# pengpeng-yu/FastPCC

Hardware: NVIDIA B200
Metric: encode+decode Mpts/s (higher is better)
Workload: dtype int8

## Files before the change

### fastpcc_b200/_lib.py

```python
import ctypes as C
import os.path as osp

from . import build as _build

_vp, _i, _i64, _sz = C.c_void_p, C.c_int, C.c_int64, C.c_size_t


class Epilogue(C.Structure):
    _fields_ = [('bias', _vp), ('slope', _vp), ('requant_mul', _vp), ('zero_point', _vp),
                ('shift', C.c_int32), ('out_type', C.c_int32), ('mul_is_scalar', C.c_int32),
                ('residual', _vp), ('post_slope', _vp), ('row_bias', _vp), ('row_idx', _vp), ('row_bias_bound', C.c_int32),
                ('post_requant_mul', _vp), ('post_zero_point', _vp), ('post_shift', C.c_int32), ('post_requant_slope', _vp), ('aux_out', _vp), ('out_ld', C.c_int64)]


_EP = C.POINTER(Epilogue)

SIGNATURES = {
    'fpcc_last_error': (C.c_char_p, []),
    'fpcc_version': (_i, []),
    'fpcc_device_check': (_i, [_vp, _vp, _vp]),
    'fpcc_hash_insert_coords': (_i, [_vp, _vp, _i, _vp, _i, _i, _vp]),
    'fpcc_kmap_lookup': (_i, [_vp, _vp, _i, _vp, _i, _i, _i, _i, _i, _i, _i, _i, _i, _vp, _i, _i64, _vp]),
    'fpcc_kmap_compact_workspace': (_sz, [_i, _i]),
    'fpcc_kmap_compact': (_i, [_vp, _i, _i, _i64, _i, _vp, _vp, _vp, _vp, _sz, _vp]),
    'fpcc_kmap_from_parent': (_i, [_vp, _i64, _i, _vp, _vp, _vp, _vp, _i, _vp, _i64, _vp]),
    'fpcc_kmap_row_masks': (_i, [_vp, _i, _i, _i64, _vp, _vp]),
    'fpcc_kmap_permute': (_i, [_vp, _i, _i, _i64, _vp, _vp, _i64, _vp]),
    'fpcc_scan_workspace': (_sz, [_i]),
    'fpcc_downsample': (_i, [_vp, _i, _vp, _vp, _vp, _vp, _vp, _vp, _sz, _vp]),
    'fpcc_upsample': (_i, [_vp, _vp, _i, _vp, _vp, _vp, _vp, _vp, _vp, _sz, _vp]),
    'fpcc_occ_to_bits': (_i, [_vp, _i, _vp, _vp]),
    'fpcc_gather_patches': (_i, [_vp, _i, _vp, _i64, _i, _i, _vp, _i, _vp]),
    'fpcc_occ_bits_q8': (_i, [_vp, _i64, _i, _i, _vp, _i64, _vp]),
    'fpcc_slot_table': (_i, [_vp, _vp, _i, _vp, _i64, _vp]),
    'fpcc_morton_encode': (_i, [_vp, _i64, _i, _i, _vp, _vp]),
    'fpcc_gather_rows16': (_i, [_vp, _vp, _i64, _vp, _vp]),
    'fpcc_voxelize_workspace': (_sz, [_i64]),
    'fpcc_voxelize_f32': (_i, [_vp, _i64, _i, C.c_float, _i, _i, _i, _vp, _vp, _vp, _vp, _sz, _vp]),
    'fpcc_kd_split_workspace': (_sz, [_i64, _i]),
    'fpcc_kd_split': (_i, [_vp, _i64, _i, _vp, _vp, _vp, _sz, _vp]),
    'fpcc_frame_header_write': (_i, [_vp, _i, _vp]),
    'fpcc_frame_header_read': (_i, [_vp, _i64, _vp, _vp]),
    'fpcc_partitions_pack': (_i64, [_vp, _vp, _i, _vp, _i64]),
    'fpcc_partitions_index': (_i, [_vp, _i64, _i, _vp, _vp]),
    'fpcc_bytes_list_concat': (_i64, [_vp, _vp, _i, _vp, _i64]),
    'fpcc_bytes_list_split': (_i64, [_vp, _i64, _i, _vp, _vp]),
    'fpcc_nn_search': (_i, [_vp, _i, _i, _i, _vp, _i, _i, _i, _i, _vp, _vp, _vp]),
    'fpcc_knn_workspace': (_sz, [_i64, _i]),
    'fpcc_knn_search': (_i, [_i, _i, _i, _vp, _i64, _i, _i, _i, _vp, _i64, _i, _i, _i, _vp, _vp, _vp, _sz, _vp]),
    'fpcc_gemm_i8': (_i, [_vp, _vp, _vp, _i, _vp, _i, _i, _i, _vp]),
# ... 64 lines not shown
```

### fastpcc_b200/csrc/coords.cu

```cuda
#include <cub/cub.cuh>

#include "common.cuh"

namespace fpcc {


__device__ __forceinline__ int4 load_bxyz(const int32_t *coords, int64_t i, int layout) {
    int4 c = reinterpret_cast<const int4 *>(coords)[i];
    return layout == 0 ? c : make_int4(c.w, c.x, c.y, c.z);
}

__global__ void __launch_bounds__(256) hash_insert_kernel(unsigned long long *keys, int32_t *vals, uint32_t capacity,
                                                          const int32_t *coords, int n, int layout) {
    int i = blockIdx.x * blockDim.x + threadIdx.x;
    if (i >= n) return;
    int4 c = load_bxyz(coords, i, layout);
    if (!coord_in_range(c.x, c.y, c.z, c.w)) return;
    unsigned long long key = pack_key(c.x, c.y, c.z, c.w);
    uint32_t slot = hash_slot(key, capacity);
    while (true) {
        unsigned long long prev = atomicCAS(&keys[slot], 0ull, key);
        if (prev == 0ull || prev == key) {
            vals[slot] = i + 1;
            return;
// ... 43 lines not shown
    }
    dx = d[0]; dy = d[1]; dz = d[2];
}

__global__ void __launch_bounds__(256) kmap_lookup_kernel(const unsigned long long *__restrict__ keys,
                                                          const int32_t *__restrict__ vals, uint32_t capacity,
                                                          const int32_t *__restrict__ out_coords, int n_out, int layout,
                                                          KernelGeom g, int32_t *__restrict__ table, int k_major, int64_t ld) {
    int o = blockIdx.x * blockDim.x + threadIdx.x;
    int k = blockIdx.y;
    if (o >= n_out) return;
    int dx, dy, dz;
    kernel_offset(g, k, dx, dy, dz);
    int4 c = load_bxyz(out_coords, o, layout);
    int x, y, z;
    if (g.me) { x = c.y + dx; y = c.z + dy; z = c.w + dz; }
    else { x = c.y * g.st[0] + dx; y = c.z * g.st[1] + dy; z = c.w * g.st[2] + dz; }
    int32_t v = 0;
    if (coord_in_range(c.x, x, y, z)) v = hash_find(keys, vals, capacity, pack_key(c.x, x, y, z));
    if (k_major) table[(int64_t)k * ld + o] = v;
    else table[(int64_t)o * g.kvol + k] = v;
}

__global__ void __launch_bounds__(256) kmap_from_parent_kernel(const int32_t *__restrict__ ctable, int64_t ldc,
                                                               const uint8_t *__restrict__ cocc, const int32_t *__restrict__ cbase,
                                                               const int32_t *__restrict__ parent, const uint8_t *__restrict__ slot,
                                                               int n_fine, int32_t *__restrict__ table, int64_t ld) {
    const int i = blockIdx.x * blockDim.x + threadIdx.x;
    if (i >= n_fine) return;
    const int j = parent[i];
    const int s = slot[i];
    const int sx = (s >> 2) & 1, sy = (s >> 1) & 1, sz = s & 1;
    uint32_t pocc[8];
    int32_t pbase[8];
#pragma unroll
    for (int q = 0; q < 8; ++q) {
        const int K = (sx + (q & 1)) + 3 * (sy + ((q >> 1) & 1)) + 9 * (sz + (q >> 2));
        const int32_t jn = __ldg(&ctable[(int64_t)K * ldc + j]);
        pocc[q] = jn ? (uint32_t)__ldg(&cocc[jn - 1]) : 0u;
        pbase[q] = jn ? __ldg(&cbase[jn - 1]) : 0;
    }
#pragma unroll
    for (int dz = -1; dz <= 1; ++dz) {
        const int tz = sz + dz;
        const bool cz = ((tz >> 1) - (sz - 1)) != 0;
        uint32_t o4[4];
        int32_t b4[4];
#pragma unroll
        for (int q = 0; q < 4; ++q) { o4[q] = cz ? pocc[4 + q] : pocc[q]; b4[q] = cz ? pbase[4 + q] : pbase[q]; }
#pragma unroll
        for (int dy = -1; dy <= 1; ++dy) {
            const int ty = sy + dy;
            const bool cy = ((ty >> 1) - (sy - 1)) != 0;
            const uint32_t o2a = cy ? o4[2] : o4[0], o2b = cy ? o4[3] : o4[1];
            const int32_t b2a = cy ? b4[2] : b4[0], b2b = cy ? b4[3] : b4[1];
#pragma unroll
            for (int dx = -1; dx <= 1; ++dx) {
                const int tx = sx + dx;
                const bool cx = ((tx >> 1) - (sx - 1)) != 0;
                const uint32_t o = cx ? o2b : o2a;
                const int32_t b = cx ? b2b : b2a;
                const int sn = ((tx & 1) << 2) | ((ty & 1) << 1) | (tz & 1);
                const int32_t v = ((o >> (7 - sn)) & 1u) ? b + __popc(o >> (8 - sn)) + 1 : 0;
                const int k = (dx + 1) + 3 * (dy + 1) + 9 * (dz + 1);
                table[(int64_t)k * ld + i] = v;
            }
        }
    }
}

__global__ void __launch_bounds__(256) kmap_row_masks_kernel(const int32_t *__restrict__ table, int kvol, int n_out, int64_t ld,
                                                             int32_t *__restrict__ masks) {
    int o = blockIdx.x * blockDim.x + threadIdx.x;
    if (o >= n_out) return;
    uint32_t m = 0;
    for (int k = 0; k < kvol; ++k) m |= (uint32_t)(table[(int64_t)k * ld + o] != 0) << (k < 31 ? k : 31);
    masks[o] = (int32_t)(m & 0x7FFFFFFFu);
}
__global__ void __launch_bounds__(256) kmap_permute_kernel(const int32_t *__restrict__ table, int n_out, int64_t ld,
                                                           const int32_t *__restrict__ perm, int32_t *__restrict__ out, int64_t ld_out) {
    int j = blockIdx.x * blockDim.x + threadIdx.x;
    int k = blockIdx.y;
    if (j >= n_out) return;
    out[(int64_t)k * ld_out + j] = table[(int64_t)k * ld + perm[j]];
}

constexpr int CHUNK = 2048;

__global__ void __launch_bounds__(256) compact_count_kernel(const int32_t *__restrict__ table, int n_out, int64_t ld,
                                                            int omit_k, int nchunks, int32_t *__restrict__ counts) {
    int k = blockIdx.y, chunk = blockIdx.x;
    int base = chunk * CHUNK;
    int c = 0;
    if (k != omit_k) {
        for (int j = threadIdx.x; j < CHUNK; j += 256) {
            int o = base + j;
            if (o < n_out && table[(int64_t)k * ld + o] != 0) ++c;
        }
    }
    typedef cub::BlockReduce<int, 256> BR;
    __shared__ typename BR::TempStorage tmp;
    int tot = BR(tmp).Sum(c);
    if (threadIdx.x == 0) counts[k * nchunks + chunk] = tot;
}

__global__ void __launch_bounds__(256) compact_write_kernel(const int32_t *__restrict__ table, int n_out, int64_t ld,
                                                            int omit_k, int nchunks, const int32_t *__restrict__ starts,
// ... 145 lines not shown
                                int32_t *table, int k_major, int64_t ld, void *stream) {
    FPCC_REQUIRE(keys && vals && out_coords && table, "kmap_lookup: NULL pointer");
    FPCC_REQUIRE(ksx > 0 && ksy > 0 && ksz > 0 && sx > 0 && sy > 0 && sz > 0, "kmap_lookup: bad kernel geometry");
    FPCC_REQUIRE(capacity > 0 && n_out >= 0, "kmap_lookup: bad sizes");
    FPCC_REQUIRE(!k_major || ld >= n_out, "kmap_lookup: ld %lld < n_out %d", (long long)ld, n_out);
    FPCC_REQUIRE(((uintptr_t)out_coords & 15) == 0, "kmap_lookup: coords must be 16-byte aligned");
    if (n_out == 0) return FPCC_OK;
    KernelGeom g;
    g.ks[0] = ksx; g.ks[1] = ksy; g.ks[2] = ksz;
    g.st[0] = sx; g.st[1] = sy; g.st[2] = sz;
    g.kvol = ksx * ksy * ksz;
    g.me = convention == 1;
    FPCC_REQUIRE(convention == 0 || convention == 1, "kmap_lookup: unknown convention");
    FPCC_REQUIRE(g.kvol <= 65535, "kmap_lookup: kernel volume too large");
    dim3 grid(ceil_div(n_out, 256), g.kvol);
    kmap_lookup_kernel<<<grid, 256, 0, (cudaStream_t)stream>>>((const unsigned long long *)keys, vals, (uint32_t)capacity,
                                                               out_coords, n_out, layout, g, table, k_major, ld);
    FPCC_LAUNCH_CHECK();
    return FPCC_OK;
}

extern "C" int fpcc_kmap_from_parent(const int32_t *coarse_table, int64_t ld_coarse, int n_coarse, const uint8_t *coarse_occ,
                                     const int32_t *child_base, const int32_t *parent, const uint8_t *slot, int n_fine,
                                     int32_t *table, int64_t ld, void *stream) {
    FPCC_REQUIRE(coarse_table && coarse_occ && child_base && parent && slot && table, "kmap_from_parent: NULL pointer");
    FPCC_REQUIRE(n_coarse > 0 && ld_coarse >= n_coarse && n_fine >= 0 && ld >= n_fine, "kmap_from_parent: bad sizes");
    if (n_fine == 0) return FPCC_OK;
    kmap_from_parent_kernel<<<ceil_div(n_fine, 256), 256, 0, (cudaStream_t)stream>>>(coarse_table, ld_coarse, coarse_occ, child_base,
                                                                                                  parent, slot, n_fine, table, ld);
    FPCC_LAUNCH_CHECK();
    return FPCC_OK;
}

extern "C" int fpcc_kmap_row_masks(const int32_t *table, int kvol, int n_out, int64_t ld, int32_t *masks, void *stream) {
    FPCC_REQUIRE(table && masks, "kmap_row_masks: NULL pointer");
    FPCC_REQUIRE(kvol > 0 && n_out >= 0 && ld >= n_out, "kmap_row_masks: bad sizes");
    if (n_out == 0) return FPCC_OK;
    kmap_row_masks_kernel<<<ceil_div(n_out, 256), 256, 0, (cudaStream_t)stream>>>(table, kvol, n_out, ld, masks);
    FPCC_LAUNCH_CHECK();
    return FPCC_OK;
}

extern "C" int fpcc_kmap_permute(const int32_t *table, int kvol, int n_out, int64_t ld, const int32_t *perm, int32_t *out,
                                 int64_t ld_out, void *stream) {
    FPCC_REQUIRE(table && perm && out, "kmap_permute: NULL pointer");
    FPCC_REQUIRE(kvol > 0 && kvol <= 65535 && n_out >= 0 && ld >= n_out && ld_out >= n_out, "kmap_permute: bad sizes");
    if (n_out == 0) return FPCC_OK;
    kmap_permute_kernel<<<dim3(ceil_div(n_out, 256), kvol), 256, 0, (cudaStream_t)stream>>>(table, n_out, ld, perm, out, ld_out);
    FPCC_LAUNCH_CHECK();
    return FPCC_OK;
}

static size_t scan_temp_bytes(int n) {
    size_t t = 0;
    cub::DeviceScan::ExclusiveSum((void *)nullptr, t, (const int32_t *)nullptr, (int32_t *)nullptr, n);
    return (t + 255) & ~(size_t)255;
}

extern "C" size_t fpcc_kmap_compact_workspace(int kvol, int n_out) {
    int nchunks = ceil_div(n_out > 0 ? n_out : 1, CHUNK);
    size_t cnt = ((size_t)kvol * nchunks * sizeof(int32_t) + 255) & ~(size_t)255;
    return 2 * cnt + scan_temp_bytes(kvol * nchunks) + 256;
}

extern "C" int fpcc_kmap_compact(const int32_t *table, int kvol, int n_out, int64_t ld, int omit_k, int32_t *in_map,
                                 int32_t *out_map, int32_t *offsets, void *workspace, size_t workspace_bytes, void *stream) {
    FPCC_REQUIRE(table && in_map && out_map && offsets && workspace, "kmap_compact: NULL pointer");
    FPCC_REQUIRE(kvol > 0 && n_out > 0 && ld >= n_out, "kmap_compact: bad sizes");
    FPCC_REQUIRE(workspace_bytes >= fpcc_kmap_compact_workspace(kvol, n_out), "kmap_compact: workspace too small");
    cudaStream_t s = (cudaStream_t)stream;
    int nchunks = ceil_div(n_out, CHUNK);
// ... 203 lines not shown
```

### fastpcc_b200/csrc/entropy.cu

```cuda
#include "common.cuh"

namespace fpcc {

constexpr int EXP_LUT_SIZE = 12 * 512 + 1;
__device__ const int32_t g_exp_lut[EXP_LUT_SIZE] = {
#include "exp_lut.inc"
};

__device__ __forceinline__ int32_t warp_max(int32_t v) {
    return __reduce_max_sync(0xffffffffu, v);
}
__device__ __forceinline__ int32_t warp_sum(int32_t v) {
    return __reduce_add_sync(0xffffffffu, v);
}

struct RowStat {
    int32_t row_max;
    uint64_t inv;
};
__device__ __forceinline__ int32_t lut_of(int32_t row_max, int32_t x) {
    int32_t id = (row_max - x) >> 7;
    return __ldg(&g_exp_lut[id > EXP_LUT_SIZE - 1 ? EXP_LUT_SIZE - 1 : id]);
}
__device__ __forceinline__ RowStat row_stat(const int32_t *__restrict__ row, int S, int pre_shift, int lane) {
    int32_t m = INT32_MIN;
    for (int j = lane; j < S; j += 32) m = max(m, row[j] >> pre_shift);
    RowStat st;
    st.row_max = warp_max(m) + 64;
// ... 36 lines not shown
#pragma unroll
            for (int d = 1; d < 32; d <<= 1) {
                uint32_t t = __shfl_up_sync(0xffffffffu, v, d);
                if (lane >= d) v += t;
            }
            uint32_t c = running + v;
            running += __shfl_sync(0xffffffffu, v, 31);
            if (j == S - 1) c = 65535;
            if (MODE == 0) {
                if (j < ld) cdf[r * ld + j] = j < S ? (uint16_t)c : (uint16_t)0xFFFF;
            } else {
                if (j == sym - 1) lo = c;
                if (j == sym) hi = (j == S - 1) ? 65536u : c;
            }
        }
        if (MODE == 1) {
            lo = __reduce_or_sync(0xffffffffu, lo);
            hi = __reduce_or_sync(0xffffffffu, hi);
            if (lane == 0) ranges[r] = lo | ((hi - lo - 1u) << 16);
        }
    }
}

template <int MODE>
__global__ void __launch_bounds__(256) cdf_row_kernel(const int32_t *__restrict__ logits, int64_t logits_ld, int64_t rows, int S,
                                                      uint16_t *__restrict__ cdf, int ld, const int32_t *__restrict__ symbols,
                                                      uint32_t *__restrict__ ranges) {
    const int lane = threadIdx.x & 31;
    const bool vec_in = (logits_ld & 3) == 0 && ((uintptr_t)logits & 15) == 0 && 8 * lane + 8 <= logits_ld;
    const bool vec_out = MODE == 0 && ld == 256 && ((uintptr_t)cdf & 15) == 0;
    const uint32_t scale = (uint32_t)(65536 - S);
    for (int64_t r = (int64_t)blockIdx.x * 8 + (threadIdx.x >> 5); r < rows; r += (int64_t)gridDim.x * 8) {
        const int32_t *row = logits + r * logits_ld;
        int32_t x[8];
        if (vec_in) {
            const int4 a = __ldg(reinterpret_cast<const int4 *>(row) + 2 * lane), b = __ldg(reinterpret_cast<const int4 *>(row) + 2 * lane + 1);
            x[0] = a.x; x[1] = a.y; x[2] = a.z; x[3] = a.w; x[4] = b.x; x[5] = b.y; x[6] = b.z; x[7] = b.w;
        } else {
#pragma unroll
            for (int i = 0; i < 8; ++i) x[i] = 8 * lane + i < S ? __ldg(&row[8 * lane + i]) : 0;
        }
        int32_t m = INT32_MIN;
#pragma unroll
        for (int i = 0; i < 8; ++i) {
            x[i] >>= 7;
            if (8 * lane + i < S) m = max(m, x[i]);
        }
        const int32_t row_max = warp_max(m) + 64;
        int32_t e[8];
        int32_t sum = 0;
#pragma unroll
        for (int i = 0; i < 8; ++i) {
            e[i] = 8 * lane + i < S ? lut_of(row_max, x[i]) : 0;
            sum += e[i];
        }
        sum = warp_sum(sum);
        uint64_t inv;
        if (sum > 0) inv = (uint64_t)__double2ull_rz(__ddiv_rn((double)((1ull << 32) + (uint64_t)(sum >> 1)), (double)sum));
        else inv = (1ull << 32) / (uint64_t)S;
        uint32_t c[8];
        uint32_t run = 0;
#pragma unroll
        for (int i = 0; i < 8; ++i) {
            const uint64_t p = (uint64_t)(uint32_t)e[i] * inv;
            const uint32_t p32 = p > 0xFFFFFFFFull ? 0xFFFFFFFFu : (uint32_t)p;
            run += 8 * lane + i < S ? __umulhi(p32, scale) + 1u : 0u;
            c[i] = run;
        }
        uint32_t incl = run;
#pragma unroll
        for (int d = 1; d < 32; d <<= 1) {
            const uint32_t t = __shfl_up_sync(0xffffffffu, incl, d);
            if (lane >= d) incl += t;
        }
        const uint32_t base = incl - run;
#pragma unroll
        for (int i = 0; i < 8; ++i) {
            c[i] += base;
            if (8 * lane + i == S - 1) c[i] = 65535u;
        }
        if (MODE == 0) {
            if (vec_out) {
                uint32_t w[4];
#pragma unroll
                for (int t = 0; t < 4; ++t) {
                    const uint32_t lo = 8 * lane + 2 * t < S ? c[2 * t] : 0xFFFFu, hi = 8 * lane + 2 * t + 1 < S ? c[2 * t + 1] : 0xFFFFu;
                    w[t] = (lo & 0xFFFFu) | (hi << 16);
                }
                reinterpret_cast<uint4 *>(cdf + r * ld)[lane] = make_uint4(w[0], w[1], w[2], w[3]);
            } else {
#pragma unroll
                for (int i = 0; i < 8; ++i)
                    if (8 * lane + i < ld) cdf[r * ld + 8 * lane + i] = 8 * lane + i < S ? (uint16_t)c[i] : (uint16_t)0xFFFF;
            }
        } else {
            int sym = symbols[r];
            sym = sym < 0 ? 0 : (sym > S - 1 ? S - 1 : sym);
            if ((sym >> 3) == lane) {
                const int si = sym & 7;
                uint32_t lo = base, hi = 0;
#pragma unroll
                for (int i = 0; i < 8; ++i) {
                    if (i == si) hi = c[i];
                    if (i + 1 == si) lo = c[i];
                }
                if (sym == S - 1) hi = 65536u;
                ranges[r] = lo | ((hi - lo - 1u) << 16);
            }
        }
    }
}

__global__ void __launch_bounds__(256) table_ranges_kernel(const uint16_t *__restrict__ cdf, int64_t n_cdf, int S,
                                                           const int32_t *__restrict__ symbols, int64_t rows,
                                                           uint32_t *__restrict__ ranges) {
    int64_t r = (int64_t)blockIdx.x * blockDim.x + threadIdx.x;
    if (r >= rows) return;
    const uint16_t *row = n_cdf == 1 ? cdf : cdf + r * S;
    int s = symbols[r];
    s = s < 0 ? 0 : (s > S - 1 ? S - 1 : s);
    uint32_t lo = s == 0 ? 0u : row[s - 1];
    uint32_t hi = s == S - 1 ? 65536u : row[s];
    ranges[r] = lo | ((hi - lo - 1u) << 16);
}

static int row_grid(int64_t rows) {
    int64_t b = (rows + 7) / 8;
    int64_t cap = (int64_t)sm_count() * 8;
    return (int)(b < cap ? b : cap);
}

}

using namespace fpcc;

extern "C" int fpcc_softmax_i32(const int32_t *in, int64_t rows, int c, uint32_t *out, void *stream) {
    FPCC_REQUIRE(in && out, "softmax_i32: NULL pointer");
    FPCC_REQUIRE(rows > 0 && c > 1 && rows * c <= 0xFFFFFFFFll, "softmax_i32: need N > 0, C > 1, N*C < 2^32");
    softmax_kernel<<<row_grid(rows), 256, 0, (cudaStream_t)stream>>>(in, rows, c, out);
    FPCC_LAUNCH_CHECK();
    return FPCC_OK;
}

extern "C" int fpcc_quantize_cdf(const int32_t *logits, int64_t logits_ld, int64_t rows, int s, uint16_t *cdf, int ld, void *stream) {
    FPCC_REQUIRE(logits && cdf, "quantize_cdf: NULL pointer");
    FPCC_REQUIRE(logits_ld >= s, "quantize_cdf: logits pitch %lld < s = %d", (long long)logits_ld, s);
    FPCC_REQUIRE(rows > 0 && s > 1 && s < 65536 && ld >= s, "quantize_cdf: bad sizes");
    if (s <= 256) cdf_row_kernel<0><<<row_grid(rows), 256, 0, (cudaStream_t)stream>>>(logits, logits_ld, rows, s, cdf, ld, nullptr, nullptr);
    else cdf_kernel<0><<<row_grid(rows), 256, 0, (cudaStream_t)stream>>>(logits, logits_ld, rows, s, cdf, ld, nullptr, nullptr);
    FPCC_LAUNCH_CHECK();
    return FPCC_OK;
}

extern "C" int fpcc_cdf_symbol_ranges(const int32_t *logits, int64_t logits_ld, int64_t rows, int s, const int32_t *symbols,
                                      uint32_t *ranges, void *stream) {
    FPCC_REQUIRE(logits && symbols && ranges, "cdf_symbol_ranges: NULL pointer");
    FPCC_REQUIRE(logits_ld >= s, "cdf_symbol_ranges: logits pitch %lld < s = %d", (long long)logits_ld, s);
    FPCC_REQUIRE(rows > 0 && s > 1 && s < 65536, "cdf_symbol_ranges: bad sizes");
    if (s <= 256) cdf_row_kernel<1><<<row_grid(rows), 256, 0, (cudaStream_t)stream>>>(logits, logits_ld, rows, s, nullptr, 0, symbols, ranges);
    else cdf_kernel<1><<<row_grid(rows), 256, 0, (cudaStream_t)stream>>>(logits, logits_ld, rows, s, nullptr, 0, symbols, ranges);
    FPCC_LAUNCH_CHECK();
    return FPCC_OK;
}

extern "C" int fpcc_table_symbol_ranges(const uint16_t *cdf, int64_t n_cdf, int s, const int32_t *symbols, int64_t rows,
                                        uint32_t *ranges, void *stream) {
    FPCC_REQUIRE(cdf && symbols && ranges, "table_symbol_ranges: NULL pointer");
    FPCC_REQUIRE(rows > 0 && s > 0 && (n_cdf == 1 || n_cdf == rows), "table_symbol_ranges: bad sizes");
    table_ranges_kernel<<<ceil_div(rows, 256), 256, 0, (cudaStream_t)stream>>>(cdf, n_cdf, s, symbols, rows, ranges);
    FPCC_LAUNCH_CHECK();
    return FPCC_OK;
}
```

### fastpcc_b200/int_sparse_conv/cuda_ops.py

```python
import math
from typing import Any, Dict, List, Optional, Tuple

import torch
import torch.nn as nn

from .. import ops
from ..sparse_tensor import SparseTensor
from . import ext as int_sparse_conv_ext

SharedFxpShift = 23
WeightRange = (1 << 7) - 1
ActRange = (1 << 7) - 1


GROUP_ROWS_MIN = 4096


class KernelMap:

    def __init__(self, table: torch.Tensor, idx_omit_map: int = -1):
        self.table = table
        self.idx_omit_map = idx_omit_map
        self._pairs = None
        self._grouped = None

    def grouped(self):
        if self._grouped is None:
            self._grouped = ops.group_rows(self.table)
        return self._grouped

    @classmethod
    def from_pair_lists(cls, in_out_maps, n_out, kernel_volume, n_in_equals_out_centre=-1, device=None):
        table = torch.zeros((kernel_volume, n_out), dtype=torch.int32, device=device)
        for k, (im, om) in enumerate(in_out_maps):
            if im is not None:
                table[k, om.long()] = im + 1
        if n_in_equals_out_centre >= 0:
            table[n_in_equals_out_centre] = torch.arange(1, n_out + 1, dtype=torch.int32, device=device)
        return cls(table, n_in_equals_out_centre)

    def as_pair_lists(self, idx_omit_map=None) -> List[Tuple[Optional[torch.Tensor], Optional[torch.Tensor]]]:
        omit = self.idx_omit_map if idx_omit_map is None else idx_omit_map
        if self._pairs is None or self._pairs[0] != omit:
            in_map, out_map, offsets = ops.kmap_compact(self.table, omit)
            off = offsets.tolist()
            maps = []
            for k in range(self.table.shape[0]):
                maps.append((None, None) if off[k + 1] == off[k] else (in_map[off[k]: off[k + 1]], out_map[off[k]: off[k + 1]]))
            self._pairs = (omit, maps)
        return self._pairs[1]

# ... 561 lines not shown
```

### fastpcc_b200/lossl_coord_int/model.py

```python
from dataclasses import dataclass
from typing import List, Optional

import numpy as np
import torch
import torch.nn as nn

from .. import bitstream, ops
from ..int_sparse_conv.cuda_ops import (
    SharedFxpShift, SparseResBlockIn32W8Out32, SparseConvIn8W8Out8, SparseConvIn8W8Out32,
    SparseConvPReLUIn8W8Out8, SparseConvPReLUIn8W8Out32, PReLUIn32Out32, RequantFxpToScaledInt8,
    LinearIn8W8Out8, LinearIn8W8Out32, LinearPReLUIn8W8Out8, LinearPReLUIn8W8Out32, LinearIn8W8, KernelMap)
from ..sparse_tensor import SparseTensor

_DENSE = (PReLUIn32Out32, RequantFxpToScaledInt8, LinearIn8W8)


@dataclass
class Config:
    channels: int = 256
    max_stride_wo_recurrent: int = 2048
    max_stride: int = 8192
    fea_stride: int = 16
    use_more_ch_for_multi_step_pred: bool = False
    skip_top_scales_num: int = 0


class _Trace:

    def __init__(self):
        import os
        self.on = os.environ.get('FPCC_TRACE', '0') == '1'
        self.t = None
        self.rows = []

# ... 71 lines not shown


def _with(f, ref: SparseTensor, C=None, stride=None):
    x = SparseTensor(f, ref.C if C is None else C, ref.stride if stride is None else stride, None)
    x._caches = ref._caches
    return x


_K3 = ((3, 3, 3), (1, 1, 1))
import os as _os
DUAL_OUTPUTS = _os.environ.get('FPCC_DUAL_OUTPUTS', '0') == '1'
CAT_BITS = _os.environ.get('FPCC_CAT_BITS', '1') != '0'


def seed_kernel_map(src_caches, dst_caches, coarse_stride, coarse_occ: torch.Tensor, fine: Level):
    if fine.parent is None or fine.slot is None or coarse_occ is None:
        return
    entry = src_caches.kmaps.get((tuple(coarse_stride),) + _K3)
    kmap = entry.get('in_out_maps') if entry is not None else None
    if not isinstance(kmap, KernelMap) or kmap.table.shape[1] != coarse_occ.shape[0]:
        return
    tag = (tuple(s // 2 for s in coarse_stride),) + _K3
    if tag not in dst_caches.kmaps:
        table = ops.kmap_from_parent(kmap.table, coarse_occ.contiguous(), fine.parent.contiguous(), fine.slot.contiguous())
        dst_caches.kmaps[tag] = {'in_out_maps': KernelMap(table)}


class OneScalePredictor(nn.Module):

    def __init__(self, channels, if_upsample=True, allow_single_ch=False):
        super().__init__()
        if allow_single_ch:
            self.dec_init = SparseConvIn8W8Out32(1, channels)
        self.dec = SparseResBlockIn32W8Out32(channels)
        self.pred = SparseSequential(
            RequantFxpToScaledInt8(), SparseConvPReLUIn8W8Out8(channels, channels), LinearIn8W8Out32(channels, 255))
        self.pred[-1].padded_output = True
        self.if_upsample = if_upsample
        if if_upsample:
            self.upsample = SparseSequential(
                RequantFxpToScaledInt8(), LinearPReLUIn8W8Out32(channels + 8, channels),
                SparseResBlockIn32W8Out32(channels), RequantFxpToScaledInt8(), LinearIn8W8Out32(channels, channels * 8))
        else:
            self.upsample = None

    def trunk(self, cur: SparseTensor):
        if cur.F.shape[1] == 1:
            cur = self.dec_init(cur)
# ... 491 lines not shown
```

### fastpcc_b200/ops.py

```python
import ctypes as C
import threading

import torch

from . import _lib
from ._lib import Epilogue

OUT_I8, OUT_I16, OUT_I32 = 0, 1, 2
_OUT_DTYPE = {OUT_I8: torch.int8, OUT_I16: torch.int16, OUT_I32: torch.int32}
CDF_LD = 256


def _s():
    return torch.cuda.current_stream().cuda_stream


def _p(t):
    return None if t is None else t.data_ptr()


def _need(t, dtype, name, dim=None):
    if t.dtype != dtype:
        raise RuntimeError(f'{name}: expected {dtype}, got {t.dtype}')
    if not t.is_cuda:
# ... 272 lines not shown
    work = ({'bytes': float(inp.numel() * 4 + inp.numel() * _OUT_DTYPE[ep.out_type].itemsize), 'desc': f'{inp.shape[0]}x{inp.shape[1]} out{ep.out_type}'}
            if _prof is not None else None)
    if out is not None and not out.is_contiguous():
        if out.dtype != torch.int8 or out.dim() != 2 or tuple(out.shape) != tuple(inp.shape) or out.stride(1) != 1:
            raise RuntimeError('requant: a strided output must be an int8 [rows, ch] column slice')
        _call('fpcc_requant_ld', _p(inp), inp.shape[0], inp.shape[1], C.byref(ep), out.data_ptr(), out.stride(0), _s(), tag='fpcc_requant', work=work)
        return out
    out = torch.empty(inp.shape, dtype=_OUT_DTYPE[ep.out_type], device=inp.device) if out is None else out
    _call('fpcc_requant', _p(inp), inp.shape[0], inp.shape[1], C.byref(ep), _p(out), _s(), work=work)
    return out


def prelu_i32(inp, slope):
    _need(inp, torch.int32, 'input', 2)
    _need(slope, torch.int32, 'slope')
    out = torch.empty_like(inp)
    _call('fpcc_prelu_i32', _p(inp), inp.numel(), _p(slope), _p(out), _s())
    return out


_POPC8 = {}


def kmap_from_parent(coarse_table, coarse_occ, parent, slot):
    _need(coarse_table, torch.int32, 'coarse table', 2)
    _need(coarse_occ, torch.uint8, 'coarse occupancy', 1)
    _need(parent, torch.int32, 'parent', 1)
    _need(slot, torch.uint8, 'slot', 1)
    if coarse_table.shape[0] != 27 or coarse_table.shape[1] != coarse_occ.shape[0] or parent.shape[0] != slot.shape[0]:
        raise RuntimeError('kmap_from_parent: shape mismatch')
    dev = coarse_table.device
    lut = _POPC8.get(dev.index)
    if lut is None:
        with cache_lock:
            lut = _POPC8.get(dev.index)
            if lut is None:
                lut = torch.tensor([bin(v).count('1') for v in range(256)], dtype=torch.int32, device=dev)
                publish_ready(dev)
                _POPC8[dev.index] = lut
    cnt = lut[coarse_occ.long()]
    base = (torch.cumsum(cnt, 0, dtype=torch.int32) - cnt).contiguous()
    n_c, n_f = coarse_occ.shape[0], parent.shape[0]
    table = torch.empty((27, n_f), dtype=torch.int32, device=dev)
    _call('fpcc_kmap_from_parent', _p(coarse_table), n_c, n_c, _p(coarse_occ), _p(base), _p(parent), _p(slot), n_f, _p(table), n_f, _s(),
          work={'bytes': 4.0 * 27 * n_f + 5.0 * n_f + 4.0 * 27 * n_c})
    return table


def _tile_offsets_of(table):
    kv, n = table.shape
    any_k = (table != 0)
    pad = (-n) % 128
    if pad:
        any_k = torch.nn.functional.pad(any_k, (0, pad))
    return float(any_k.view(kv, -1, 128).any(dim=2).sum().item())


def group_rows(table):
    _need(table, torch.int32, 'table', 2)
    kv, n_out = table.shape
    masks = torch.empty(n_out, dtype=torch.int32, device=table.device)
    _call('fpcc_kmap_row_masks', _p(table), kv, n_out, n_out, _p(masks), _s(), work={'bytes': 4.0 * kv * n_out + 4.0 * n_out})
    perm = torch.sort(masks, stable=True)[1].to(torch.int32)
    table_p = torch.empty_like(table)
    _call('fpcc_kmap_permute', _p(table), kv, n_out, n_out, _p(perm), _p(table_p), n_out, _s(), work={'bytes': 8.0 * kv * n_out + 4.0 * n_out})
    return table_p, perm


def spconv(in_feats, weight, table, ep, zp_comp=None, out=None, row_perm=None):
    _need(in_feats, torch.int8, 'in_feats', 2)
    _need(weight, torch.int8, 'weight', 3)
    _need(table, torch.int32, 'table', 2)
    kv, c_out, c_in = weight.shape
    if table.shape[0] != kv or in_feats.shape[1] != c_in:
        raise RuntimeError(f'spconv: shape mismatch weight {tuple(weight.shape)} table {tuple(table.shape)} feats {tuple(in_feats.shape)}')
    n_out = table.shape[1]
    out = torch.empty((n_out, c_out), dtype=_ep_out_dtype(ep), device=in_feats.device) if out is None else out
    tag = work = None
    if _prof is not None:
        tag = 'spconv_' + gemm_engine(c_in, c_out, kv, zp_comp is not None)
        pairs = _pairs_of(table)
        work = {'ops': 2.0 * pairs * c_in * c_out, 'mma_ops': 2.0 * ((n_out + 127) // 128 * 128) * kv * c_in * c_out,
                'exec_ops': 2.0 * 128 * _tile_offsets_of(table) * c_in * c_out,
                'bytes': float(in_feats.numel() + weight.numel() + out.numel() * out.element_size() + 4 * table.numel())}
    if row_perm is not None:
        _need(row_perm, torch.int32, 'row_perm', 1)
        if row_perm.numel() != n_out:
            raise RuntimeError('spconv: row_perm must have one entry per output row')
# ... 250 lines not shown
```

### include/fastpcc_b200.h

```cpp
#ifndef FASTPCC_B200_H_
#define FASTPCC_B200_H_

#include <stddef.h>
#include <stdint.h>

#ifdef __cplusplus
extern "C" {
#endif

#define FPCC_OK 0
#define FPCC_ERR_INVALID (-1)
#define FPCC_ERR_CUDA (-2)
#define FPCC_ERR_UNSUPPORTED (-3)

#define FPCC_OUT_I8 0
#define FPCC_OUT_I16 1
#define FPCC_OUT_I32 2

const char *fpcc_last_error(void);
int fpcc_version(void);
int fpcc_device_check(int *cc_major, int *cc_minor, int *sm_count);


int fpcc_hash_insert_coords(int64_t *keys, int32_t *vals, int capacity,
                            const int32_t *coords, int n, int layout, void *stream);

int fpcc_kmap_lookup(const int64_t *keys, const int32_t *vals, int capacity,
                     const int32_t *out_coords, int n_out, int layout,
                     int ksx, int ksy, int ksz, int sx, int sy, int sz, int convention,
                     int32_t *table, int k_major, int64_t ld, void *stream);

size_t fpcc_kmap_compact_workspace(int kvol, int n_out);
int fpcc_kmap_compact(const int32_t *table, int kvol, int n_out, int64_t ld, int omit_k,
                      int32_t *in_map, int32_t *out_map, int32_t *offsets ,
                      void *workspace, size_t workspace_bytes, void *stream);

int fpcc_kmap_from_parent(const int32_t *coarse_table, int64_t ld_coarse, int n_coarse, const uint8_t *coarse_occ,
                          const int32_t *child_base, const int32_t *parent, const uint8_t *slot, int n_fine,
                          int32_t *table, int64_t ld, void *stream);

int fpcc_kmap_row_masks(const int32_t *table, int kvol, int n_out, int64_t ld, int32_t *masks, void *stream);
int fpcc_kmap_permute(const int32_t *table, int kvol, int n_out, int64_t ld, const int32_t *perm, int32_t *out,
                      int64_t ld_out, void *stream);

size_t fpcc_scan_workspace(int n);
int fpcc_downsample(const int32_t *coords, int n, int32_t *out_coords, uint8_t *out_occ,
                    int32_t *parent_of_child, uint8_t *slot_of_child, int32_t *n_out_dev,
                    void *workspace, size_t workspace_bytes, void *stream);

int fpcc_upsample(const int32_t *coords, const uint8_t *occ, int n,
                  int32_t *child_coords, int32_t *child_parent, uint8_t *child_slot, int32_t *n_child_dev,
                  const int32_t *shift_add, void *workspace, size_t workspace_bytes, void *stream);

int fpcc_occ_to_bits(const uint8_t *occ, int n, int32_t *bits_i32 , void *stream);

int fpcc_morton_encode(const int32_t *xyz, int64_t ld, int n, int msb_axis, int64_t *codes, void *stream);
int fpcc_gather_rows16(const void *src, const int64_t *idx, int64_t n, void *dst, void *stream);

size_t fpcc_voxelize_workspace(int64_t n);
int fpcc_voxelize_f32(const float *points, int64_t n, int ld, float scale, int coord_bits, int msb_axis, int batch,
                      int32_t *out_coords, float *min_xyz_dev, int32_t *n_out_dev, void *workspace,
                      size_t workspace_bytes, void *stream);

size_t fpcc_kd_split_workspace(int64_t n, int coord_bits);
int fpcc_kd_split(const int32_t *coords, int64_t n, int coord_bits, int32_t *out_coords, int32_t *info_dev,
                  void *workspace, size_t workspace_bytes, void *stream);
// ... 138 lines not shown
```

Baseline: 24.70.

## Fuse row masks and row-major copy into kmap_from_parent; stage exp LUT in smem

kmap_from_parent can now also write a row-major copy of the kernel map and per-row occupancy masks through a shared-memory tile. The later grouping step uses these masks instead of running a separate mask kernel, and a new warp-transposing permute kernel reads the contiguous rows instead of doing strided gathers from the k-major table. Separately, the CDF row kernel copies the exp LUT into shared memory, pads tail lanes to remove per-element bounds checks, and sizes its grid from occupancy. This trades extra global writes (the row copy) and shared-memory use for fewer kernel launches and better-coalesced permutation reads.

```diff
diff --git a/fastpcc_b200/_lib.py b/fastpcc_b200/_lib.py
--- a/fastpcc_b200/_lib.py
+++ b/fastpcc_b200/_lib.py
@@ -23,9 +23,10 @@
     'fpcc_kmap_lookup': (_i, [_vp, _vp, _i, _vp, _i, _i, _i, _i, _i, _i, _i, _i, _i, _vp, _i, _i64, _vp]),
     'fpcc_kmap_compact_workspace': (_sz, [_i, _i]),
     'fpcc_kmap_compact': (_i, [_vp, _i, _i, _i64, _i, _vp, _vp, _vp, _vp, _sz, _vp]),
-    'fpcc_kmap_from_parent': (_i, [_vp, _i64, _i, _vp, _vp, _vp, _vp, _i, _vp, _i64, _vp]),
+    'fpcc_kmap_from_parent': (_i, [_vp, _i64, _i, _vp, _vp, _vp, _vp, _i, _vp, _i64, _vp, _vp, _vp]),
     'fpcc_kmap_row_masks': (_i, [_vp, _i, _i, _i64, _vp, _vp]),
     'fpcc_kmap_permute': (_i, [_vp, _i, _i, _i64, _vp, _vp, _i64, _vp]),
+    'fpcc_kmap_permute_rows': (_i, [_vp, _i, _i, _vp, _vp, _i64, _vp]),
     'fpcc_scan_workspace': (_sz, [_i]),
     'fpcc_downsample': (_i, [_vp, _i, _vp, _vp, _vp, _vp, _vp, _vp, _sz, _vp]),
     'fpcc_upsample': (_i, [_vp, _vp, _i, _vp, _vp, _vp, _vp, _vp, _vp, _sz, _vp]),
diff --git a/fastpcc_b200/csrc/coords.cu b/fastpcc_b200/csrc/coords.cu
--- a/fastpcc_b200/csrc/coords.cu
+++ b/fastpcc_b200/csrc/coords.cu
@@ -89,24 +89,29 @@
     else table[(int64_t)o * g.kvol + k] = v;
 }
 
-__global__ void __launch_bounds__(256) kmap_from_parent_kernel(const int32_t *__restrict__ ctable, int64_t ldc,
-                                                               const uint8_t *__restrict__ cocc, const int32_t *__restrict__ cbase,
-                                                               const int32_t *__restrict__ parent, const uint8_t *__restrict__ slot,
-                                                               int n_fine, int32_t *__restrict__ table, int64_t ld) {
-    const int i = blockIdx.x * blockDim.x + threadIdx.x;
-    if (i >= n_fine) return;
-    const int j = parent[i];
-    const int s = slot[i];
+constexpr int KFP_THREADS = 256;
+__global__ void __launch_bounds__(KFP_THREADS) kmap_from_parent_kernel(const int32_t *__restrict__ ctable, int64_t ldc,
+                                                                       const uint8_t *__restrict__ cocc, const int32_t *__restrict__ cbase,
+                                                                       const int32_t *__restrict__ parent, const uint8_t *__restrict__ slot,
+                                                                       int n_fine, int32_t *__restrict__ table, int64_t ld,
+                                                                       int32_t *__restrict__ rows, int32_t *__restrict__ masks) {
+    extern __shared__ __align__(16) int32_t kfp_tile[];
+    const int i0 = blockIdx.x * KFP_THREADS;
+    const int i = i0 + threadIdx.x;
+    const bool live = i < n_fine;
+    const int j = live ? parent[i] : 0;
+    const int s = live ? slot[i] : 0;
     const int sx = (s >> 2) & 1, sy = (s >> 1) & 1, sz = s & 1;
     uint32_t pocc[8];
     int32_t pbase[8];
 #pragma unroll
     for (int q = 0; q < 8; ++q) {
         const int K = (sx + (q & 1)) + 3 * (sy + ((q >> 1) & 1)) + 9 * (sz + (q >> 2));
-        const int32_t jn = __ldg(&ctable[(int64_t)K * ldc + j]);
+        const int32_t jn = live ? __ldg(&ctable[(int64_t)K * ldc + j]) : 0;
         pocc[q] = jn ? (uint32_t)__ldg(&cocc[jn - 1]) : 0u;
         pbase[q] = jn ? __ldg(&cbase[jn - 1]) : 0;
     }
+    uint32_t mask = 0;
 #pragma unroll
     for (int dz = -1; dz <= 1; ++dz) {
         const int tz = sz + dz;
@@ -130,10 +135,20 @@
                 const int sn = ((tx & 1) << 2) | ((ty & 1) << 1) | (tz & 1);
                 const int32_t v = ((o >> (7 - sn)) & 1u) ? b + __popc(o >> (8 - sn)) + 1 : 0;
                 const int k = (dx + 1) + 3 * (dy + 1) + 9 * (dz + 1);
-                table[(int64_t)k * ld + i] = v;
+                if (live) table[(int64_t)k * ld + i] = v;
+                if (rows) kfp_tile[threadIdx.x * 27 + k] = v;
+                mask |= (uint32_t)(v != 0) << k;
             }
         }
     }
+    if (!rows) return;
+    if (live) masks[i] = (int32_t)mask;
+    __syncthreads();
+    const int n_words = min(KFP_THREADS, n_fine - i0) * 27;
+    int32_t *dst = rows + (int64_t)i0 * 27;
+    for (int w = threadIdx.x; w < n_words / 4; w += KFP_THREADS)
+        reinterpret_cast<int4 *>(dst)[w] = reinterpret_cast<const int4 *>(kfp_tile)[w];
+    for (int w = (n_words & ~3) + threadIdx.x; w < n_words; w += KFP_THREADS) dst[w] = kfp_tile[w];
 }
 
 __global__ void __launch_bounds__(256) kmap_row_masks_kernel(const int32_t *__restrict__ table, int kvol, int n_out, int64_t ld,
@@ -150,6 +165,28 @@
     int k = blockIdx.y;
     if (j >= n_out) return;
     out[(int64_t)k * ld_out + j] = table[(int64_t)k * ld + perm[j]];
+}
+constexpr int KPR_PITCH = 33;
+__global__ void __launch_bounds__(256) kmap_permute_rows_kernel(const int32_t *__restrict__ rows, int kvol, int n_out,
+                                                                const int32_t *__restrict__ perm, int32_t *__restrict__ out, int64_t ld_out) {
+    __shared__ int32_t tiles[8][32 * KPR_PITCH];
+    const int lane = threadIdx.x & 31, warp = threadIdx.x >> 5;
+    const int j0 = (blockIdx.x * 8 + warp) * 32;
+    if (j0 >= n_out) return;
+    const int nr = min(32, n_out - j0);
+    const int p = lane < nr ? __ldg(&perm[j0 + lane]) : 0;
+    int32_t v[32];
+#pragma unroll
+    for (int r = 0; r < 32; ++r) {
+        const int src = __shfl_sync(0xffffffffu, p, r);
+        v[r] = r < nr && lane < kvol ? __ldg(&rows[(int64_t)src * kvol + lane]) : 0;
+    }
+    int32_t *t = tiles[warp];
+#pragma unroll
+    for (int r = 0; r < 32; ++r) t[r * KPR_PITCH + lane] = v[r];
+    __syncwarp();
+    if (lane < nr)
+        for (int k = 0; k < kvol; ++k) out[(int64_t)k * ld_out + j0 + lane] = t[lane * KPR_PITCH + k];
 }
 
 constexpr int CHUNK = 2048;
@@ -341,12 +378,15 @@
 
 extern "C" int fpcc_kmap_from_parent(const int32_t *coarse_table, int64_t ld_coarse, int n_coarse, const uint8_t *coarse_occ,
                                      const int32_t *child_base, const int32_t *parent, const uint8_t *slot, int n_fine,
-                                     int32_t *table, int64_t ld, void *stream) {
+                                     int32_t *table, int64_t ld, int32_t *rows, int32_t *masks, void *stream) {
     FPCC_REQUIRE(coarse_table && coarse_occ && child_base && parent && slot && table, "kmap_from_parent: NULL pointer");
+    FPCC_REQUIRE(!rows == !masks, "kmap_from_parent: rows and masks go together");
+    FPCC_REQUIRE(!rows || ((uintptr_t)rows & 15) == 0, "kmap_from_parent: rows must be 16-byte aligned");
     FPCC_REQUIRE(n_coarse > 0 && ld_coarse >= n_coarse && n_fine >= 0 && ld >= n_fine, "kmap_from_parent: bad sizes");
     if (n_fine == 0) return FPCC_OK;
-    kmap_from_parent_kernel<<<ceil_div(n_fine, 256), 256, 0, (cudaStream_t)stream>>>(coarse_table, ld_coarse, coarse_occ, child_base,
-                                                                                                  parent, slot, n_fine, table, ld);
+    const size_t smem = rows ? (size_t)KFP_THREADS * 27 * sizeof(int32_t) : 0;
+    kmap_from_parent_kernel<<<ceil_div(n_fine, KFP_THREADS), KFP_THREADS, smem, (cudaStream_t)stream>>>(
+        coarse_table, ld_coarse, coarse_occ, child_base, parent, slot, n_fine, table, ld, rows, masks);
     FPCC_LAUNCH_CHECK();
     return FPCC_OK;
 }
@@ -366,6 +406,16 @@
     FPCC_REQUIRE(kvol > 0 && kvol <= 65535 && n_out >= 0 && ld >= n_out && ld_out >= n_out, "kmap_permute: bad sizes");
     if (n_out == 0) return FPCC_OK;
     kmap_permute_kernel<<<dim3(ceil_div(n_out, 256), kvol), 256, 0, (cudaStream_t)stream>>>(table, n_out, ld, perm, out, ld_out);
+    FPCC_LAUNCH_CHECK();
+    return FPCC_OK;
+}
+
+extern "C" int fpcc_kmap_permute_rows(const int32_t *rows, int kvol, int n_out, const int32_t *perm, int32_t *out, int64_t ld_out,
+                                      void *stream) {
+    FPCC_REQUIRE(rows && perm && out, "kmap_permute_rows: NULL pointer");
+    FPCC_REQUIRE(kvol > 0 && kvol <= 32 && n_out >= 0 && ld_out >= n_out, "kmap_permute_rows: bad sizes");
+    if (n_out == 0) return FPCC_OK;
+    kmap_permute_rows_kernel<<<ceil_div(n_out, 256), 256, 0, (cudaStream_t)stream>>>(rows, kvol, n_out, perm, out, ld_out);
     FPCC_LAUNCH_CHECK();
     return FPCC_OK;
 }
diff --git a/fastpcc_b200/csrc/entropy.cu b/fastpcc_b200/csrc/entropy.cu
--- a/fastpcc_b200/csrc/entropy.cu
+++ b/fastpcc_b200/csrc/entropy.cu
@@ -3,7 +3,7 @@
 namespace fpcc {
 
 constexpr int EXP_LUT_SIZE = 12 * 512 + 1;
-__device__ const int32_t g_exp_lut[EXP_LUT_SIZE] = {
+__device__ __align__(16) const int32_t g_exp_lut[EXP_LUT_SIZE] = {
 #include "exp_lut.inc"
 };
 
@@ -86,15 +86,23 @@
     }
 }
 
+constexpr int32_t CDF_PAD = -(1 << 30);
 template <int MODE>
 __global__ void __launch_bounds__(256) cdf_row_kernel(const int32_t *__restrict__ logits, int64_t logits_ld, int64_t rows, int S,
                                                       uint16_t *__restrict__ cdf, int ld, const int32_t *__restrict__ symbols,
                                                       uint32_t *__restrict__ ranges) {
+    __shared__ __align__(16) int32_t lut[EXP_LUT_SIZE];
+    for (int i = threadIdx.x; i < (EXP_LUT_SIZE - 1) / 4; i += blockDim.x)
+        reinterpret_cast<int4 *>(lut)[i] = reinterpret_cast<const int4 *>(g_exp_lut)[i];
+    if (threadIdx.x == 0) lut[EXP_LUT_SIZE - 1] = g_exp_lut[EXP_LUT_SIZE - 1];
+    __syncthreads();
     const int lane = threadIdx.x & 31;
     const bool vec_in = (logits_ld & 3) == 0 && ((uintptr_t)logits & 15) == 0 && 8 * lane + 8 <= logits_ld;
     const bool vec_out = MODE == 0 && ld == 256 && ((uintptr_t)cdf & 15) == 0;
+    const bool tail = 8 * lane + 8 > S - 1;
     const uint32_t scale = (uint32_t)(65536 - S);
     for (int64_t r = (int64_t)blockIdx.x * 8 + (threadIdx.x >> 5); r < rows; r += (int64_t)gridDim.x * 8) {
+        int sym = MODE == 1 ? __ldg(&symbols[r]) : 0;
         const int32_t *row = logits + r * logits_ld;
         int32_t x[8];
         if (vec_in) {
@@ -104,31 +112,31 @@
 #pragma unroll
             for (int i = 0; i < 8; ++i) x[i] = 8 * lane + i < S ? __ldg(&row[8 * lane + i]) : 0;
         }
-        int32_t m = INT32_MIN;
+#pragma unroll
+        for (int i = 0; i < 8; ++i) x[i] >>= 7;
+        if (tail) {
+#pragma unroll
+            for (int i = 0; i < 8; ++i)
+                if (8 * lane + i >= S) x[i] = CDF_PAD;
+        }
+        int32_t m = max(max(max(x[0], x[1]), max(x[2], x[3])), max(max(x[4], x[5]), max(x[6], x[7])));
+        const int32_t row_max = warp_max(m) + 64;
+        uint32_t e[8];
+        uint32_t sum = 0;
 #pragma unroll
         for (int i = 0; i < 8; ++i) {
-            x[i] >>= 7;
-            if (8 * lane + i < S) m = max(m, x[i]);
-        }
-        const int32_t row_max = warp_max(m) + 64;
-        int32_t e[8];
-        int32_t sum = 0;
-#pragma unroll
-        for (int i = 0; i < 8; ++i) {
-            e[i] = 8 * lane + i < S ? lut_of(row_max, x[i]) : 0;
+            e[i] = (uint32_t)lut[min((row_max - x[i]) >> 7, EXP_LUT_SIZE - 1)];
             sum += e[i];
         }
-        sum = warp_sum(sum);
-        uint64_t inv;
-        if (sum > 0) inv = (uint64_t)__double2ull_rz(__ddiv_rn((double)((1ull << 32) + (uint64_t)(sum >> 1)), (double)sum));
-        else inv = (1ull << 32) / (uint64_t)S;
+        sum = (uint32_t)warp_sum((int32_t)sum);
+        const uint32_t inv = (uint32_t)__double2ull_rz(__ddiv_rn((double)((1ull << 32) + (uint64_t)(sum >> 1)), (double)sum));
         uint32_t c[8];
         uint32_t run = 0;
 #pragma unroll
         for (int i = 0; i < 8; ++i) {
-            const uint64_t p = (uint64_t)(uint32_t)e[i] * inv;
-            const uint32_t p32 = p > 0xFFFFFFFFull ? 0xFFFFFFFFu : (uint32_t)p;
-            run += 8 * lane + i < S ? __umulhi(p32, scale) + 1u : 0u;
+            const uint64_t p = (uint64_t)e[i] * inv;
+            const uint32_t p32 = (p >> 32) ? 0xFFFFFFFFu : (uint32_t)p;
+            run += __umulhi(p32, scale) + 1u;
             c[i] = run;
         }
         uint32_t incl = run;
@@ -139,26 +147,24 @@
         }
         const uint32_t base = incl - run;
 #pragma unroll
-        for (int i = 0; i < 8; ++i) {
-            c[i] += base;
-            if (8 * lane + i == S - 1) c[i] = 65535u;
-        }
+        for (int i = 0; i < 8; ++i) c[i] += base;
         if (MODE == 0) {
+            if (tail) {
+#pragma unroll
+                for (int i = 0; i < 8; ++i)
+                    if (8 * lane + i >= S - 1) c[i] = 0xFFFFu;
+            }
             if (vec_out) {
                 uint32_t w[4];
 #pragma unroll
-                for (int t = 0; t < 4; ++t) {
-                    const uint32_t lo = 8 * lane + 2 * t < S ? c[2 * t] : 0xFFFFu, hi = 8 * lane + 2 * t + 1 < S ? c[2 * t + 1] : 0xFFFFu;
-                    w[t] = (lo & 0xFFFFu) | (hi << 16);
-                }
+                for (int t = 0; t < 4; ++t) w[t] = (c[2 * t] & 0xFFFFu) | (c[2 * t + 1] << 16);
                 reinterpret_cast<uint4 *>(cdf + r * ld)[lane] = make_uint4(w[0], w[1], w[2], w[3]);
             } else {
 #pragma unroll
                 for (int i = 0; i < 8; ++i)
-                    if (8 * lane + i < ld) cdf[r * ld + 8 * lane + i] = 8 * lane + i < S ? (uint16_t)c[i] : (uint16_t)0xFFFF;
+                    if (8 * lane + i < ld) cdf[r * ld + 8 * lane + i] = (uint16_t)c[i];
             }
         } else {
-            int sym = symbols[r];
             sym = sym < 0 ? 0 : (sym > S - 1 ? S - 1 : sym);
             if ((sym >> 3) == lane) {
                 const int si = sym & 7;
@@ -194,6 +200,18 @@
     return (int)(b < cap ? b : cap);
 }
 
+template <int MODE>
+static int cdf_row_grid(int64_t rows) {
+    static int per_sm = 0;
+    if (per_sm == 0) {
+        int n = 0;
+        if (cudaOccupancyMaxActiveBlocksPerMultiprocessor(&n, cdf_row_kernel<MODE>, 256, 0) != cudaSuccess || n < 1) n = 1;
+        per_sm = n;
+    }
+    const int64_t b = (rows + 31) / 32, cap = (int64_t)sm_count() * per_sm;
+    return (int)(b < cap ? b : cap);
+}
+
 }
 
 using namespace fpcc;
@@ -210,7 +228,7 @@
     FPCC_REQUIRE(logits && cdf, "quantize_cdf: NULL pointer");
     FPCC_REQUIRE(logits_ld >= s, "quantize_cdf: logits pitch %lld < s = %d", (long long)logits_ld, s);
     FPCC_REQUIRE(rows > 0 && s > 1 && s < 65536 && ld >= s, "quantize_cdf: bad sizes");
-    if (s <= 256) cdf_row_kernel<0><<<row_grid(rows), 256, 0, (cudaStream_t)stream>>>(logits, logits_ld, rows, s, cdf, ld, nullptr, nullptr);
+    if (s <= 256) cdf_row_kernel<0><<<cdf_row_grid<0>(rows), 256, 0, (cudaStream_t)stream>>>(logits, logits_ld, rows, s, cdf, ld, nullptr, nullptr);
     else cdf_kernel<0><<<row_grid(rows), 256, 0, (cudaStream_t)stream>>>(logits, logits_ld, rows, s, cdf, ld, nullptr, nullptr);
     FPCC_LAUNCH_CHECK();
     return FPCC_OK;
@@ -221,7 +239,7 @@
     FPCC_REQUIRE(logits && symbols && ranges, "cdf_symbol_ranges: NULL pointer");
     FPCC_REQUIRE(logits_ld >= s, "cdf_symbol_ranges: logits pitch %lld < s = %d", (long long)logits_ld, s);
     FPCC_REQUIRE(rows > 0 && s > 1 && s < 65536, "cdf_symbol_ranges: bad sizes");
-    if (s <= 256) cdf_row_kernel<1><<<row_grid(rows), 256, 0, (cudaStream_t)stream>>>(logits, logits_ld, rows, s, nullptr, 0, symbols, ranges);
+    if (s <= 256) cdf_row_kernel<1><<<cdf_row_grid<1>(rows), 256, 0, (cudaStream_t)stream>>>(logits, logits_ld, rows, s, nullptr, 0, symbols, ranges);
     else cdf_kernel<1><<<row_grid(rows), 256, 0, (cudaStream_t)stream>>>(logits, logits_ld, rows, s, nullptr, 0, symbols, ranges);
     FPCC_LAUNCH_CHECK();
     return FPCC_OK;
diff --git a/fastpcc_b200/int_sparse_conv/cuda_ops.py b/fastpcc_b200/int_sparse_conv/cuda_ops.py
--- a/fastpcc_b200/int_sparse_conv/cuda_ops.py
+++ b/fastpcc_b200/int_sparse_conv/cuda_ops.py
@@ -18,15 +18,17 @@
 
 class KernelMap:
 
-    def __init__(self, table: torch.Tensor, idx_omit_map: int = -1):
+    def __init__(self, table: torch.Tensor, idx_omit_map: int = -1, rows=None, masks=None):
         self.table = table
         self.idx_omit_map = idx_omit_map
         self._pairs = None
         self._grouped = None
+        self._rows, self._masks = rows, masks
 
     def grouped(self):
         if self._grouped is None:
-            self._grouped = ops.group_rows(self.table)
+            self._grouped = ops.group_rows(self.table, self._rows, self._masks)
+            self._rows = self._masks = None
         return self._grouped
 
     @classmethod
diff --git a/fastpcc_b200/lossl_coord_int/model.py b/fastpcc_b200/lossl_coord_int/model.py
--- a/fastpcc_b200/lossl_coord_int/model.py
+++ b/fastpcc_b200/lossl_coord_int/model.py
@@ -9,7 +9,7 @@
 from ..int_sparse_conv.cuda_ops import (
     SharedFxpShift, SparseResBlockIn32W8Out32, SparseConvIn8W8Out8, SparseConvIn8W8Out32,
     SparseConvPReLUIn8W8Out8, SparseConvPReLUIn8W8Out32, PReLUIn32Out32, RequantFxpToScaledInt8,
-    LinearIn8W8Out8, LinearIn8W8Out32, LinearPReLUIn8W8Out8, LinearPReLUIn8W8Out32, LinearIn8W8, KernelMap)
+    LinearIn8W8Out8, LinearIn8W8Out32, LinearPReLUIn8W8Out8, LinearPReLUIn8W8Out32, LinearIn8W8, KernelMap, GROUP_ROWS_MIN)
 from ..sparse_tensor import SparseTensor
 
 _DENSE = (PReLUIn32Out32, RequantFxpToScaledInt8, LinearIn8W8)
@@ -127,8 +127,12 @@
         return
     tag = (tuple(s // 2 for s in coarse_stride),) + _K3
     if tag not in dst_caches.kmaps:
-        table = ops.kmap_from_parent(kmap.table, coarse_occ.contiguous(), fine.parent.contiguous(), fine.slot.contiguous())
-        dst_caches.kmaps[tag] = {'in_out_maps': KernelMap(table)}
+        args = (kmap.table, coarse_occ.contiguous(), fine.parent.contiguous(), fine.slot.contiguous())
+        if fine.n >= GROUP_ROWS_MIN:
+            table, rows, masks = ops.kmap_from_parent(*args, with_rows=True)
+            dst_caches.kmaps[tag] = {'in_out_maps': KernelMap(table, rows=rows, masks=masks)}
+        else:
+            dst_caches.kmaps[tag] = {'in_out_maps': KernelMap(ops.kmap_from_parent(*args))}
 
 
 class OneScalePredictor(nn.Module):
diff --git a/fastpcc_b200/ops.py b/fastpcc_b200/ops.py
--- a/fastpcc_b200/ops.py
+++ b/fastpcc_b200/ops.py
@@ -318,7 +318,7 @@
 _POPC8 = {}
 
 
-def kmap_from_parent(coarse_table, coarse_occ, parent, slot):
+def kmap_from_parent(coarse_table, coarse_occ, parent, slot, with_rows=False):
     _need(coarse_table, torch.int32, 'coarse table', 2)
     _need(coarse_occ, torch.uint8, 'coarse occupancy', 1)
     _need(parent, torch.int32, 'parent', 1)
@@ -338,9 +338,14 @@
     base = (torch.cumsum(cnt, 0, dtype=torch.int32) - cnt).contiguous()
     n_c, n_f = coarse_occ.shape[0], parent.shape[0]
     table = torch.empty((27, n_f), dtype=torch.int32, device=dev)
-    _call('fpcc_kmap_from_parent', _p(coarse_table), n_c, n_c, _p(coarse_occ), _p(base), _p(parent), _p(slot), n_f, _p(table), n_f, _s(),
-          work={'bytes': 4.0 * 27 * n_f + 5.0 * n_f + 4.0 * 27 * n_c})
-    return table
+    rows = masks = None
+    if with_rows:
+        rows = torch.empty((n_f, 27), dtype=torch.int32, device=dev)
+        masks = torch.empty(n_f, dtype=torch.int32, device=dev)
+    _call('fpcc_kmap_from_parent', _p(coarse_table), n_c, n_c, _p(coarse_occ), _p(base), _p(parent), _p(slot), n_f, _p(table), n_f,
+          _p(rows), _p(masks), _s(),
+          work={'bytes': (8.0 * 27 + 4.0 if with_rows else 4.0 * 27) * n_f + 5.0 * n_f + 4.0 * 27 * n_c})
+    return (table, rows, masks) if with_rows else table
 
 
 def _tile_offsets_of(table):
@@ -352,14 +357,22 @@
     return float(any_k.view(kv, -1, 128).any(dim=2).sum().item())
 
 
-def group_rows(table):
+def group_rows(table, rows=None, masks=None):
     _need(table, torch.int32, 'table', 2)
     kv, n_out = table.shape
-    masks = torch.empty(n_out, dtype=torch.int32, device=table.device)
-    _call('fpcc_kmap_row_masks', _p(table), kv, n_out, n_out, _p(masks), _s(), work={'bytes': 4.0 * kv * n_out + 4.0 * n_out})
+    if masks is None:
+        masks = torch.empty(n_out, dtype=torch.int32, device=table.device)
+        _call('fpcc_kmap_row_masks', _p(table), kv, n_out, n_out, _p(masks), _s(), work={'bytes': 4.0 * kv * n_out + 4.0 * n_out})
     perm = torch.sort(masks, stable=True)[1].to(torch.int32)
     table_p = torch.empty_like(table)
-    _call('fpcc_kmap_permute', _p(table), kv, n_out, n_out, _p(perm), _p(table_p), n_out, _s(), work={'bytes': 8.0 * kv * n_out + 4.0 * n_out})
+    if rows is None:
+        _call('fpcc_kmap_permute', _p(table), kv, n_out, n_out, _p(perm), _p(table_p), n_out, _s(), work={'bytes': 8.0 * kv * n_out + 4.0 * n_out})
+    else:
+        _need(rows, torch.int32, 'rows', 2)
+        if tuple(rows.shape) != (n_out, kv) or tuple(masks.shape) != (n_out,):
+            raise RuntimeError('group_rows: rows / masks do not match the table')
+        _call('fpcc_kmap_permute_rows', _p(rows), kv, n_out, _p(perm), _p(table_p), n_out, _s(), tag='fpcc_kmap_permute',
+              work={'bytes': 8.0 * kv * n_out + 4.0 * n_out})
     return table_p, perm
 
 
diff --git a/include/fastpcc_b200.h b/include/fastpcc_b200.h
--- a/include/fastpcc_b200.h
+++ b/include/fastpcc_b200.h
@@ -37,11 +37,13 @@
 
 int fpcc_kmap_from_parent(const int32_t *coarse_table, int64_t ld_coarse, int n_coarse, const uint8_t *coarse_occ,
                           const int32_t *child_base, const int32_t *parent, const uint8_t *slot, int n_fine,
-                          int32_t *table, int64_t ld, void *stream);
+                          int32_t *table, int64_t ld, int32_t *rows, int32_t *masks, void *stream);
 
 int fpcc_kmap_row_masks(const int32_t *table, int kvol, int n_out, int64_t ld, int32_t *masks, void *stream);
 int fpcc_kmap_permute(const int32_t *table, int kvol, int n_out, int64_t ld, const int32_t *perm, int32_t *out,
                       int64_t ld_out, void *stream);
+int fpcc_kmap_permute_rows(const int32_t *rows, int kvol, int n_out, const int32_t *perm, int32_t *out, int64_t ld_out,
+                           void *stream);
 
 size_t fpcc_scan_workspace(int n);
 int fpcc_downsample(const int32_t *coords, int n, int32_t *out_coords, uint8_t *out_occ,
```

After: 24.82, median of 6. Within noise of the previous version (+0.5%).
